# NOC-OI/ship-track-estimators

Hardware: AMD Instinct MI355X
Metric: UKF+URTSS track-steps/sec (dim=4, 500-step tracks) (higher is better)
Workload: dtype f64

## Files before the change

### include/ste.h

```cpp
#ifndef STE_H
#define STE_H

#include <stdint.h>

#ifdef __cplusplus
extern "C" {
#endif

#define STE_VERSION 340

#define STE_OK 0
#define STE_EINVAL (-1)
#define STE_ELAUNCH (-2)
#define STE_ENOGPU (-3)

#define STE_FLAG_SHARED_P0 0x1u
#define STE_FLAG_NO_INITIAL_UPDATE 0x2u
#define STE_FLAG_LANES_1 0x10u
#define STE_FLAG_LANES_4 0x20u
#define STE_FLAG_PACKED_COV 0x40u
#define STE_FLAG_ROBUST 0x4u

#define STE_RTS_WORK_ROWS 30
#define STE_SLICE_ALIGN 64

#define STE_STATUS_NAN 0x1
#define STE_STATUS_CLAMPED 0x2
#define STE_STATUS_NOCONV 0x4
#define STE_STATUS_ROBUST_CAP 0x8
#define STE_STATUS_HOST_INDEX 0x10
#define STE_STATUS_BAD_INDEX 0x20

typedef struct ste_ukf_batch_f64 {
    int32_t B;
    int32_t Nmax;
    int32_t Tmax;
    int32_t n;
    uint32_t flags;
    int32_t tuning;
#define STE_TUNING_EIG_GAINS 0x100
#define STE_TUNING_TWO_KERNEL_SMOOTHER 0x200
#define STE_TUNING_ONE_KERNEL_SMOOTHER 0x400
#define STE_TUNING_LANE_RECURRENCE 0x800

    double fan_scale;
    double w0;
    double wi;

    const double* H;
    const double* Q;
    const double* R;

    const int32_t* nsteps;
    const double* x0;
    const double* P0;

    const double* dt;
    const double* sog_rate;
    const double* cog_rate;
    const double* sog_rate_rts;
    const double* cog_rate_rts;
    const int32_t* upd_idx;
    const double* z;

    const double* noise_pred;
    const double* noise_upd;
    const double* noise_rts;

    double* fwd_mean;
    double* fwd_cov;
    double* sm_mean;
    double* sm_cov;
    int32_t* status;

    double* rts_work;

    double chi_alpha;
    int32_t robust_max_iter;
    int32_t reserved2;

    int64_t track_stride;

    double* sm_pos;

    int32_t step_begin;
    int32_t step_end;
} ste_ukf_batch_f64;

int ste_version(void);

const char* ste_last_error(void);

int ste_device_count(void);

int ste_ukf_forward_f64(const ste_ukf_batch_f64* b, void* stream);

// ... 180 lines not shown
```

### ship-track-estimators_amd/csrc/ste_kernels.hip

```cpp
#include <hip/hip_runtime.h>

#include <algorithm>
#include <cstddef>
#include <cstdint>
#include <cstdio>
#include <cstring>
#include <type_traits>
#include <vector>

#include "../../include/ste.h"
#include "ste_err.h"
#include "ste_ukf.h"
#include "ste_quad.h"

namespace ste {

__shared__ int g_sched_word[2];
__device__ __forceinline__ int sched_k0() { return *(volatile int*)&g_sched_word[0]; }

template <bool kWarm>
__device__ __forceinline__ int sigma_fan(const double (&x)[4], const double (&P)[4][4], double scale,
                                         double (&sig)[9][4], EigBasis& basis);

__device__ __forceinline__ int sigma_fan(const double (&x)[4], const double (&P)[4][4], double scale,
// ... 910 lines not shown
            double Pb[4][4], D[4][4], Pbi[4][4], K[4][4];
            weighted_outer<true>(dk, dk, p.m.w0, p.m.wi, Pb);
            STE_UNROLL
            for (int r = 0; r < 4; ++r) {
                STE_UNROLL
                for (int c = 0; c < 4; ++c) Pb[r][c] += track_Q(r, c);
            }
            weighted_outer<false>(sig0, db, p.m.w0, p.m.wi, D);
            st |= sym_pinv4<true>(Pb, Pbi, pb_basis);
            pb_basis.valid = true;
            mm(D, Pbi, K);
            double y[4];
            STE_UNROLL
            for (int c = 0; c < 4; ++c) y[c] = xs[c] - xb[c];
            y[3] = wrap180(y[3]);
            STE_UNROLL
            for (int r = 0; r < 4; ++r) {
                double acc = xk[r];
                STE_UNROLL
                for (int c = 0; c < 4; ++c) acc = fma(K[r][c], y[c], acc);
                xs[r] = acc;
            }
            xs[3] = floored_mod(xs[3], 360.0);
            double dP[4][4], KdP[4][4], U[4][4];
            STE_UNROLL
            for (int r = 0; r < 4; ++r) {
                STE_UNROLL
                for (int c = 0; c < 4; ++c) dP[r][c] = Ps[r][c] - Pb[r][c];
            }
            mm(K, dP, KdP);
            mmt_sym(KdP, K, U);
            STE_UNROLL
            for (int r = 0; r < 4; ++r) {
                STE_UNROLL
                for (int c = 0; c < 4; ++c) Ps[r][c] = Pk[r][c] + U[r][c];
            }
            store_vec(p.sm_mean, (size_t)k, B, t, xs);
            store_cov_m(p.sm_cov, packed, (size_t)k, B, t, Ps);
            store_pos(p, (size_t)k, B, t, xs);
        }
    }
    if (!all_finite(xs, Ps)) st |= STE_STATUS_NAN;
    if (st) atomicOr(&p.status[t], st);
}

__device__ __forceinline__ bool work_row_full(const KParams& p, int k, int ui, bool always_full) {
    return always_full || (ui >= 0 && ui < p.Tmax) || (k == 0 && !(p.flags & STE_FLAG_NO_INITIAL_UPDATE));
}

struct RecurRow {
    double D2[8], xk[4], Pk[10];
    double shift[2];
};
template <bool kShift>
__device__ __forceinline__ void load_recur_row(const KParams& p, size_t k, size_t B, size_t t, bool d_rows23, RecurRow& g) {
    g.shift[0] = g.shift[1] = 0.0;
    if (kShift) {
        const double dt = p.dt[k * B + t];
        if (p.sog_rate_rts) g.shift[0] = (p.sog_rate_rts[k * B + t] - p.sog_rate[k * B + t]) * dt;
        if (p.cog_rate_rts) g.shift[1] = (p.cog_rate_rts[k * B + t] - p.cog_rate[k * B + t]) * dt;
    }
    const double* w = p.rts_work + (k * kWorkElems) * B + t;
    STE_UNROLL
    for (int e = 0; e < 4; ++e) g.D2[e] = w[(kWorkD + e) * B];
    if (d_rows23) {
        STE_UNROLL
        for (int e = 4; e < 8; ++e) g.D2[e] = w[(kWorkD + e) * B];
    }
    load_vec(p.fwd_mean, k, B, t, g.xk);
    load_cov_p(p.fwd_cov, (p.flags & STE_FLAG_PACKED_COV) != 0, k, B, t, g.Pk);
}

template <bool kShift, bool kTrackNoise = false>
__device__ __forceinline__ int smoother_step_gain(const KParams& p, int k, size_t B, size_t t, const RecurRow& cur,
                                                  const double (&xn)[4], const double (&Pn)[10], bool full, bool always_full,
                                                  bool all_eig, double kappa, double first_bad, double (&xb)[4],
                                                  double (&Pb)[10], double (&K)[4][4], const double* q4 = nullptr) {
    STE_UNROLL
    for (int c = 0; c < 4; ++c) xb[c] = xn[c];
    if (kShift) {
        xb[2] += cur.shift[0];
        xb[3] += cur.shift[1];
    }
    {
        double bv[4];
        STE_UNROLL
        for (int c = 0; c < 4; ++c) bv[c] = xb[c] - cur.xk[c];
        STE_UNROLL
        for (int r = 0; r < 4; ++r) {
            STE_UNROLL
            for (int c = r; c < 4; ++c) Pb[tix(r, c)] = fma(bv[r], bv[c], Pn[tix(r, c)]);
        }
    }
    if (full) {
        const double* w = p.rts_work + ((size_t)k * kWorkElems) * B + t;
        STE_UNROLL
        for (int c = 0; c < 4; ++c) xb[c] = w[(kWorkXb + c) * B];
        STE_UNROLL
        for (int e = 0; e < 10; ++e) Pb[e] = w[(kWorkPb + e) * B];
        if (kShift) {
            double bv[4];
            STE_UNROLL
            for (int c = 0; c < 4; ++c) bv[c] = xb[c] - cur.xk[c];
            if (p.noise_rts) {
                STE_UNROLL
                for (int c = 0; c < 4; ++c) bv[c] -= p.noise_rts[((size_t)k * 4 + c) * B + t];
            }
            const double s2 = cur.shift[0], s3 = cur.shift[1];
            Pb[tix(0, 2)] = fma(bv[0], s2, Pb[tix(0, 2)]);
            Pb[tix(1, 2)] = fma(bv[1], s2, Pb[tix(1, 2)]);
            Pb[tix(0, 3)] = fma(bv[0], s3, Pb[tix(0, 3)]);
            Pb[tix(1, 3)] = fma(bv[1], s3, Pb[tix(1, 3)]);
            Pb[tix(2, 2)] = fma(bv[2] + bv[2] + s2, s2, Pb[tix(2, 2)]);
            Pb[tix(3, 3)] = fma(bv[3] + bv[3] + s3, s3, Pb[tix(3, 3)]);
            Pb[tix(2, 3)] = fma(bv[2], s3, fma(s2, bv[3] + s3, Pb[tix(2, 3)]));
            xb[2] += s2;
            xb[3] += s3;
        }
    }
    double D[4][4];
    STE_UNROLL
    for (int r = 0; r < 4; ++r) {
        D[r][0] = cur.D2[r * 2 + 0];
        D[r][1] = cur.D2[r * 2 + 1];
        D[r][2] = kappa * cur.Pk[tix(r, 2)];
        D[r][3] = kappa * cur.Pk[tix(r, 3)];
    }
    if (!always_full) {
        double bv[4];
        STE_UNROLL
        for (int c = 0; c < 4; ++c) bv[c] = xb[c] - cur.xk[c];
        STE_UNROLL
        for (int r = 2; r < 4; ++r) {
            STE_UNROLL
            for (int c = 0; c < 2; ++c) {
                const double pm = full ? fma(-bv[c], bv[r], Pb[tix(c, r)]) : Pn[tix(c, r)];
                if constexpr (kTrackNoise)
                    D[r][c] = pm - q4[c * 2 + (r - 2)];
                else
                    D[r][c] = pm - p.m.Q[c * 4 + r];
            }
        }
    }
    if (__builtin_expect(__any((double)k >= first_bad), 0)) {
        if ((double)k >= first_bad) {
            const double* w = p.rts_work + ((size_t)k * kWorkElems) * B + t;
            STE_UNROLL
            for (int r = 0; r < 4; ++r) {
                D[r][2] = w[(kWorkD23 + r * 2 + 0) * B];
                D[r][3] = w[(kWorkD23 + r * 2 + 1) * B];
            }
        }
    }
    return smoother_gain(Pb, D, all_eig, K);

}

__device__ __forceinline__ void track_q4(const KParams& p, const NoiseParams& nz, size_t B, size_t t, double (&q4)[4]) {
    STE_UNROLL
    for (int c = 0; c < 2; ++c) {
        STE_UNROLL
        for (int r = 2; r < 4; ++r) q4[c * 2 + (r - 2)] = nz.Q ? nz.Q[(size_t)tix(c, r) * B + t] : p.m.Q[c * 4 + r];
    }
}

template <bool kShift, bool kTrackNoise = false>
__device__ __forceinline__ void smooth_tile_l1(const KParams& p, const size_t t, const NoiseParams* nz = nullptr) {
    const size_t B = (size_t)p.ld;
    if (t >= (size_t)p.B) return;
    double q4[4] = {0.0, 0.0, 0.0, 0.0};
    if constexpr (kTrackNoise) track_q4(p, *nz, B, t, q4);
    const int ns = p.nsteps ? p.nsteps[t] : p.Nmax;
    const bool always_full = p.noise_pred || p.noise_upd || p.noise_rts;
    const bool all_eig = (p.tuning & STE_TUNING_EIG_GAINS) != 0;
    const double kappa = (p.m.wi + p.m.wi) * p.m.fan_scale;
    const double first_bad = p.first_bad[t];
    const int last_row = p.Nmax > 0 ? p.Nmax - 1 : 0;
    auto clampk = [&](int k) -> int { return min(max(k, 0), last_row); };

    double xs[4], Ps[10], xn[4], Pn[10];
    const bool packed = (p.flags & STE_FLAG_PACKED_COV) != 0;
    load_vec(p.fwd_mean, (size_t)ns, B, t, xs);
    load_cov_p(p.fwd_cov, packed, (size_t)ns, B, t, Ps);
    store_vec(p.sm_mean, (size_t)ns, B, t, xs);
    store_cov_p(p.sm_cov, packed, (size_t)ns, B, t, Ps);
    store_pos(p, (size_t)ns, B, t, xs);
    STE_UNROLL
    for (int c = 0; c < 4; ++c) xn[c] = xs[c];
    STE_UNROLL
    for (int e = 0; e < 10; ++e) Pn[e] = Ps[e];

    RecurRow nxt;
    int ui_n = -1;
    if (ns > 0) {
        load_recur_row<kShift>(p, (size_t)(ns - 1), B, t, always_full, nxt);
        ui_n = p.upd_idx[(size_t)(ns - 1) * B + t];
    }
    int st = 0;
    for (int k = p.Nmax - 1; k >= 0; --k) {
        if (!__any(k < ns)) continue;
        if (k < ns) {
            const RecurRow cur = nxt;
            const bool full = work_row_full(p, k, ui_n, always_full);
            double xb[4], Pb[10], K[4][4];
            st |= smoother_step_gain<kShift, kTrackNoise>(p, k, B, t, cur, xn, Pn, full, always_full, all_eig, kappa, first_bad, xb, Pb, K, q4);
            {
                const int kn = clampk(k - 1);
                load_recur_row<kShift>(p, (size_t)kn, B, t, always_full, nxt);
                ui_n = p.upd_idx[(size_t)kn * B + t];
            }
            double y[4];
            STE_UNROLL
            for (int c = 0; c < 4; ++c) y[c] = xs[c] - xb[c];
            y[3] = wrap180(y[3]);
            STE_UNROLL
            for (int r = 0; r < 4; ++r) {
                double acc = cur.xk[r];
                STE_UNROLL
                for (int c = 0; c < 4; ++c) acc = fma(K[r][c], y[c], acc);
                xs[r] = acc;
            }
            xs[3] = floored_mod(xs[3], 360.0);
            double dP[10];
            STE_UNROLL
            for (int e = 0; e < 10; ++e) dP[e] = Ps[e] - Pb[e];
            double KdP[4][4];
            STE_UNROLL
            for (int r = 0; r < 4; ++r) {
                STE_UNROLL
                for (int c = 0; c < 4; ++c) {
                    double acc = K[r][0] * dP[tix(0, c)];
                    STE_UNROLL
                    for (int i = 1; i < 4; ++i) acc = fma(K[r][i], dP[tix(i, c)], acc);
                    KdP[r][c] = acc;
                }
            }
            STE_UNROLL
            for (int r = 0; r < 4; ++r) {
                STE_UNROLL
                for (int c = r; c < 4; ++c) {
                    double acc = KdP[r][0] * K[c][0];
                    STE_UNROLL
                    for (int i = 1; i < 4; ++i) acc = fma(KdP[r][i], K[c][i], acc);
                    Ps[tix(r, c)] = cur.Pk[tix(r, c)] + acc;
                }
            }
            store_vec(p.sm_mean, (size_t)k, B, t, xs);
            store_cov_p(p.sm_cov, packed, (size_t)k, B, t, Ps);
            store_pos(p, (size_t)k, B, t, xs);
            STE_UNROLL
            for (int c = 0; c < 4; ++c) xn[c] = cur.xk[c];
            STE_UNROLL
            for (int e = 0; e < 10; ++e) Pn[e] = cur.Pk[e];
        }
    }
    double chk = 0.0;
    STE_UNROLL
    for (int c = 0; c < 4; ++c) chk += xs[c] * 0.0;
    STE_UNROLL
    for (int e = 0; e < 10; ++e) chk += Ps[e] * 0.0;
    if (!(chk == 0.0)) st |= STE_STATUS_NAN;
    if (st) atomicOr(&p.status[t], st);
}

template <bool kShift>
__global__ __launch_bounds__(64) void urtss_recur_l1(const KParams p) {
    smooth_tile_l1<kShift>(p, (size_t)blockIdx.x * 64 + threadIdx.x);
}
template <bool kShift>
__global__ __launch_bounds__(64) void urtss_recur_tn(const KParams p, const NoiseParams nz) {
    smooth_tile_l1<kShift, true>(p, (size_t)blockIdx.x * 64 + threadIdx.x, &nz);
}

struct SmoothItem {
    int kp;
    int tile;
    int prog;
    int need;
};
struct SmoothSchedParams {
    const KParams* kps;
    const SmoothItem* items;
    const int* progress;
    int* error;
    unsigned long long timeout_ticks;
};
template <bool kShift>
__global__ __launch_bounds__(64) void urtss_recur_sched(const SmoothSchedParams sp) {
    typedef const KParams __attribute__((address_space(4))) ConstKParams;
    const SmoothItem* ip = sp.items + blockIdx.x;
    const int kp = __builtin_amdgcn_readfirstlane(ip->kp), tile = __builtin_amdgcn_readfirstlane(ip->tile);
    const int prog = __builtin_amdgcn_readfirstlane(ip->prog), need = __builtin_amdgcn_readfirstlane(ip->need);
    if (__hip_atomic_load(sp.error, __ATOMIC_RELAXED, __HIP_MEMORY_SCOPE_AGENT) != 0 ||
        !sched_wait(sp.progress + prog, need, sp.timeout_ticks)) {
        if (threadIdx.x == 0) __hip_atomic_store(sp.error, 2, __ATOMIC_RELAXED, __HIP_MEMORY_SCOPE_AGENT);
        return;
    }
    const KParams& p = *(const KParams*)(ConstKParams*)(uintptr_t)(sp.kps + kp);
    smooth_tile_l1<kShift>(p, (size_t)tile * 64 + threadIdx.x);
}



constexpr int kLeanK01 = kWorkD, kLeanK23 = kWorkD23;

template <bool kShift, bool kTrackNoise>
__global__ __launch_bounds__(64) void urtss_gains_all(const KParams p, const NoiseParams nz) {
    const size_t B = (size_t)p.ld;
    const size_t g = (size_t)blockIdx.x * 64 + threadIdx.x;
    if (g >= (size_t)p.B * (size_t)p.Nmax) return;
    const size_t t = g % (size_t)p.B;
    const int k = (int)(g / (size_t)p.B);
    const int ns = p.nsteps ? p.nsteps[t] : p.Nmax;
    if (k >= ns) return;
    const double fb_raw = p.first_bad[t];
    if (fb_raw < 0.0) return;
    const bool always_full = p.noise_pred || p.noise_upd || p.noise_rts;
    const bool all_eig = (p.tuning & STE_TUNING_EIG_GAINS) != 0;
    const double kappa = (p.m.wi + p.m.wi) * p.m.fan_scale;
    const bool packed = (p.flags & STE_FLAG_PACKED_COV) != 0;
    RecurRow cur;
    load_recur_row<kShift>(p, (size_t)k, B, t, always_full, cur);
    double xn[4], Pn[10];
    load_vec(p.fwd_mean, (size_t)k + 1, B, t, xn);
    load_cov_p(p.fwd_cov, packed, (size_t)k + 1, B, t, Pn);
    const bool full = work_row_full(p, k, p.upd_idx[(size_t)k * B + t], always_full);
    double xb[4], Pb[10], K[4][4], q4[4] = {0.0, 0.0, 0.0, 0.0};
    if constexpr (kTrackNoise) track_q4(p, nz, B, t, q4);
    const int st = smoother_step_gain<kShift, kTrackNoise>(p, k, B, t, cur, xn, Pn, full, always_full, all_eig, kappa, fb_raw, xb, Pb, K, q4);
    double* w = p.rts_work + ((size_t)k * kWorkElems) * B + t;
    STE_UNROLL
    for (int r = 0; r < 4; ++r) {
        w[(kLeanK01 + 2 * r + 0) * B] = K[r][0];
        w[(kLeanK01 + 2 * r + 1) * B] = K[r][1];
        w[(kLeanK23 + 2 * r + 0) * B] = K[r][2];
        w[(kLeanK23 + 2 * r + 1) * B] = K[r][3];
    }
    STE_UNROLL
    for (int c = 0; c < 4; ++c) w[(kWorkXb + c) * B] = xb[c];
    STE_UNROLL
    for (int e = 0; e < 10; ++e) w[(kWorkPb + e) * B] = Pb[e];
    if (st) atomicOr(&p.status[t], st);
}

struct LeanRow {
    double K[4][4], xb[4], Pb[10], xk[4], Pk[10];
};
__device__ __forceinline__ void load_lean_row(const KParams& p, size_t k, size_t B, size_t t, bool packed, LeanRow& g) {
    const double* w = p.rts_work + (k * kWorkElems) * B + t;
    STE_UNROLL
    for (int r = 0; r < 4; ++r) {
        g.K[r][0] = w[(kLeanK01 + 2 * r + 0) * B];
// ... 671 lines not shown
        if (kp->noise_rts) kp->noise_rts += r0 * 4 * ld;
        kp->fwd_mean += r0 * 4 * ld;
        kp->fwd_cov += r0 * (packed ? 10 : 16) * ld;
        if (kp->rts_work) kp->rts_work += r0 * STE_RTS_WORK_ROWS * ld;
    }
    return STE_OK;
}

template <class F>
auto with_bool(bool v, F&& f) {
    return v ? f(std::true_type{}) : f(std::false_type{});
}

template <class F>
auto with_forward_variant(const ste::KParams& kp, F&& f) {
    return with_bool(kp.rts_work != nullptr, [&](auto gains) {
        if (kp.fast_upd && kp.m.robust_iters > 0) return f(gains, std::true_type{}, std::true_type{});
        if (kp.fast_upd) return f(gains, std::true_type{}, std::false_type{});
        return f(gains, std::false_type{}, std::false_type{});
    });
}
int forward_variant(const ste::KParams& kp) {
    return with_forward_variant(kp, [](auto gains, auto fast, auto robust) { return gains() | fast() << 1 | robust() << 2; });
}

int launch_forward(const char* fn, const ste::KParams& kp, const ste::LikParams* lp, const ste::NoiseParams* np, hipStream_t s) {
    if (ste::choose_lanes(kp.B, kp.flags) == 4)
        return ste::launch_forward_q4(kp, s);
    const bool hist = kp.fwd_mean != nullptr;
    if (!hist && kp.rts_work) return fail(STE_EINVAL, "%s: rts_work needs the histories", fn);
    const dim3 grid((unsigned)((kp.B + 63) / 64)), block(64);
    const ste::LikParams l0 = lp ? *lp : ste::LikParams{nullptr, nullptr, nullptr, nullptr};
    with_forward_variant(kp, [&](auto gains, auto fast, auto robust) {
        constexpr bool kG = decltype(gains)::value, kF = decltype(fast)::value, kR = decltype(robust)::value;
        auto launch = [&](auto lik) {
            constexpr int kLik = decltype(lik)::value;
            if (np)
                hipLaunchKernelGGL((ste::ukf_forward_tn<kG, kF, kR, kLik>), grid, block, 0, s, kp, l0, *np);
            else if constexpr (kLik != ste::kLikOff)
                hipLaunchKernelGGL((ste::ukf_forward_lik<kG, kF, kR, kLik>), grid, block, 0, s, kp, l0);
            else
                hipLaunchKernelGGL((ste::ukf_forward_l1<kG, kF, kR>), grid, block, 0, s, kp);
        };
        if (!lp)
            launch(std::integral_constant<int, ste::kLikOff>{});
        else if (hist)
            launch(std::integral_constant<int, ste::kLikHist>{});
        else if constexpr (!kG)
            launch(std::integral_constant<int, ste::kLikOnly>{});
    });
    return check_hip(hipGetLastError(), np ? "ukf_forward_tn launch" : lp ? "ukf_forward_lik launch" : "ukf_forward launch");
}

constexpr int kLeanSmootherMaxTracks = 4096;
bool lean_smoother(const ste::KParams& kp) {
    return kp.rts_work && kp.Nmax > 0 && ((kp.tuning & STE_TUNING_TWO_KERNEL_SMOOTHER) || (!(kp.tuning & STE_TUNING_ONE_KERNEL_SMOOTHER) && kp.B <= kLeanSmootherMaxTracks));
}

int launch_backward(const ste::KParams& kp, const ste::NoiseParams* np, hipStream_t s) {
    const dim3 grid((unsigned)((kp.B + 63) / 64)), block(64);
    const bool shift = kp.sog_rate_rts || kp.cog_rate_rts, tn = np && np->Q;
    const ste::NoiseParams nz = tn ? *np : ste::NoiseParams{nullptr, nullptr};
    auto with_shift_tn = [&](auto&& f) { with_bool(shift, [&](auto sh) { with_bool(tn, [&](auto t) { f(sh, t); }); }); };
    if (lean_smoother(kp)) {
        const dim3 ggrid((unsigned)(((size_t)kp.B * (size_t)kp.Nmax + 63) / 64));
        with_shift_tn([&](auto sh, auto t) {
            hipLaunchKernelGGL((ste::urtss_gains_all<decltype(sh)::value, decltype(t)::value>), ggrid, block, 0, s, kp, nz);
        });
        int rc = check_hip(hipGetLastError(), "urtss_gains_all launch");
        if (rc) return rc;
        if (kp.tuning & STE_TUNING_LANE_RECURRENCE)
            hipLaunchKernelGGL(ste::urtss_recur_lean, grid, block, 0, s, kp);
        else
            hipLaunchKernelGGL(ste::urtss_recur_lean_q4, dim3((unsigned)((kp.B + 15) / 16)), block, 0, s, kp);
        return check_hip(hipGetLastError(), "urtss_recur_lean launch");
    }
    if (kp.rts_work) {
        with_shift_tn([&](auto sh, auto t) {
            if constexpr (decltype(t)::value)
                hipLaunchKernelGGL(ste::urtss_recur_tn<decltype(sh)::value>, grid, block, 0, s, kp, nz);
            else
                hipLaunchKernelGGL(ste::urtss_recur_l1<decltype(sh)::value>, grid, block, 0, s, kp);
        });
        return check_hip(hipGetLastError(), "urtss_recur launch");
    }
    with_bool(tn, [&](auto t) { hipLaunchKernelGGL(ste::urtss_backward_l1<decltype(t)::value>, grid, block, 0, s, kp, nz); });
    return check_hip(hipGetLastError(), "urtss_backward launch");
}

int noise_params(const char* fn, const ste_ukf_batch_f64* b, const ste_ukf_noise_f64* nz, ste::NoiseParams* np) {
    if (!b) return fail(STE_EINVAL, "batch pointer is NULL");
    if (!nz) return fail(STE_EINVAL, "%s: the per-track noise (nz) is NULL", fn);
    if (!nz->Q && !nz->R)
        return fail(STE_EINVAL, "%s: nz->Q and nz->R are both NULL: that is the plain call (without the _noise suffix)", fn);
    if (nz->flags & ~(uint32_t)STE_NOISE_R_BLOCK2) return fail(STE_EINVAL, "%s: unknown bits in nz->flags", fn);
    if (b->flags & STE_FLAG_LANES_4)
        return fail(STE_EINVAL, "%s: the quad forward kernel has no per-track noise: STE_FLAG_LANES_4 is refused", fn);
    np->Q = nz->Q;
    np->R = nz->R;
    return STE_OK;
}
void noise_route(const ste_ukf_batch_f64* b, const ste_ukf_noise_f64* nz, ste::KParams* kp) {
    kp->flags |= STE_FLAG_LANES_1;
    if (!nz->R) return;
    bool sel = true;
    for (int r = 0; r < 4; ++r)
        for (int c = 0; c < 4; ++c) sel = sel && b->H[r * 4 + c] == ((r == c && r < 2) ? 1.0 : 0.0);
    kp->fast_upd = sel && (nz->flags & STE_NOISE_R_BLOCK2) != 0;
}

int whole_passes(const char* fn, const ste_ukf_batch_f64* b, const char* why) {
    if (b->step_begin == 0 && (b->step_end == 0 || b->step_end == b->Nmax)) return STE_OK;
    snprintf(g_err, sizeof(g_err), "%s runs whole passes: %s", fn, why);
    return STE_EINVAL;
}

int lik_params(const char* fn, const ste_ukf_batch_f64* b, const ste_ukf_loglik_f64* l, ste::LikParams* lp, bool* hist) {
    if (!l) return fail(STE_EINVAL, "%s: the likelihood outputs (l) are NULL", fn);
    if (!l->loglik) return fail(STE_EINVAL, "%s: l->loglik is required", fn);
    *hist = b->fwd_mean != nullptr;
    if (*hist != (b->fwd_cov != nullptr))
        return fail(STE_EINVAL, "%s: fwd_mean and fwd_cov go together: both (histories) or neither (the likelihood alone)", fn);
    if (!*hist && b->rts_work)
        return fail(STE_EINVAL, "%s: rts_work needs the histories (the smoother reads both); pass fwd_mean and fwd_cov, or no "
                                "rts_work", fn);
    if (b->flags & STE_FLAG_LANES_4)
        return fail(STE_EINVAL, "%s runs the lane-per-track mapping only: STE_FLAG_LANES_4 is refused", fn);
    *lp = {l->loglik, l->dof, l->nupd, l->nis};
    return whole_passes(fn, b, "the likelihood sums over every update, so time slices (step_begin / step_end) are refused");
}

size_t align16(size_t v) { return (v + 15) & ~(size_t)15; }

struct SchedLayout {
    size_t kps, items, progress, total;
// ... 231 lines not shown
    sp.kps = (const ste::KParams*)(dw + lay.kps);
    sp.items = (const ste::SchedItem*)(dw + lay.items);
    sp.nrounds = sc->nrounds;
    sp.nwaves = sc->nwaves;
    sp.progress = (int*)(dw + lay.progress);
    sp.window_done = sc->window_done;
    sp.error = sc->error;
    sp.timeout_ticks = (unsigned long long)((sc->timeout_s > 0 ? sc->timeout_s : 2.0) * 1e8);
    sp.started = sc->started;
    const dim3 grid((unsigned)sc->nwaves), block(64);
    if (!first) return fail(STE_EINVAL, "scheduled forward pass: no kernel variant");
    with_forward_variant(*first, [&](auto gains, auto fast, auto robust) {
        hipLaunchKernelGGL((ste::ukf_forward_sched<decltype(gains)::value, decltype(fast)::value, decltype(robust)::value>), grid, block,
                           0, s, sp);
    });
    return check_hip(hipGetLastError(), "ukf_forward_sched launch");
}

int ste_stream_wait_counter(const int32_t* counter, int32_t need, int32_t* error, double timeout_s, void* stream) {
    if (!counter) return fail(STE_EINVAL, "counter is NULL");
    hipLaunchKernelGGL(ste::sched_gate, dim3(1), dim3(64), 0, (hipStream_t)stream, (const int*)counter, (int)need, (int*)error,
                       (unsigned long long)((timeout_s > 0 ? timeout_s : 2.0) * 1e8));
    return check_hip(hipGetLastError(), "sched_gate launch");
}

size_t ste_ukf_forward_sched_progress_offset(int32_t nwindows, int32_t max_slices, int64_t ntiles_total, int32_t nrounds,
                                             int32_t nwaves) {
    if (nwindows < 0 || max_slices < 0 || ntiles_total < 0 || nrounds < 0 || nwaves < 0) return 0;
    return sched_layout((size_t)nwindows * ((size_t)max_slices * ((size_t)max_slices + 1) / 2), (size_t)nrounds * (size_t)nwaves,
                        (size_t)ntiles_total).progress;
}

size_t ste_urtss_backward_sched_workspace(int32_t nwindows, int64_t ntiles_total) {
    if (nwindows < 0 || ntiles_total < 0) return 0;
    return align16((size_t)nwindows * sizeof(ste::KParams)) + align16((size_t)ntiles_total * sizeof(ste::SmoothItem));
}

int ste_urtss_backward_sched_f64(const ste_bwd_sched_f64* sc, void* stream) {
    if (!sc) return fail(STE_EINVAL, "schedule pointer is NULL");
    if (sc->nwindows < 1 || !sc->windows) return fail(STE_EINVAL, "scheduled smoother: nwindows >= 1 and windows are required");
    if (sc->nitems < 1 || !sc->items) return fail(STE_EINVAL, "scheduled smoother: nitems >= 1 and items are required");
    if (!sc->host_ws || !sc->dev_ws || !sc->progress || !sc->error)
        return fail(STE_EINVAL, "scheduled smoother: host_ws, dev_ws, progress and error are required");
    const int step = sc->slice_steps ? sc->slice_steps : STE_SLICE_ALIGN;
    if (step < STE_SLICE_ALIGN || step % STE_SLICE_ALIGN != 0)
        return fail(STE_EINVAL, "scheduled smoother: slice_steps must be a positive multiple of STE_SLICE_ALIGN (64)");
    const size_t kp_bytes = align16((size_t)sc->nwindows * sizeof(ste::KParams));
    const size_t total = kp_bytes + align16((size_t)sc->nitems * sizeof(ste::SmoothItem));
    if (sc->ws_bytes < total) return fail(STE_EINVAL, "scheduled smoother: workspace too small (ste_urtss_backward_sched_workspace)");
    char* hw = (char*)sc->host_ws;
    ste::KParams* kps = (ste::KParams*)hw;
    std::vector<int> nslices((size_t)sc->nwindows), tile0((size_t)sc->nwindows + 1);
    size_t ntiles = 0;
    int shift = -1;
    for (int w = 0; w < sc->nwindows; ++w) {
        const ste_ukf_batch_f64& b = sc->windows[w];
        if (b.B <= 0 || b.Nmax <= 0) return fail(STE_EINVAL, "scheduled smoother: a window has B <= 0 or Nmax <= 0");
        if (b.step_begin != 0 || b.step_end != 0) return fail(STE_EINVAL, "scheduled smoother: windows must not carry a step range of their own");
        int rc = make_params(&b, true, kps + w);
        if (rc) return rc;
        const ste::KParams& kp = kps[w];
        if (!kp.rts_work || lean_smoother(kp))
            return fail(STE_EINVAL, "scheduled smoother: every window must take the one-kernel smoother (rts_work, more than 4096 tracks or tuning bit 10)");
        const int sh = (kp.sog_rate_rts || kp.cog_rate_rts) ? 1 : 0;
        if (shift >= 0 && sh != shift) return fail(STE_EINVAL, "scheduled smoother: the windows must agree on smoother rates (one kernel runs them all)");
        shift = sh;
        nslices[w] = std::max(1, (b.Nmax + step - 1) / step);
        tile0[w] = (int)ntiles;
        ntiles += ((size_t)b.B + 63) / 64;
        if (ntiles > 0x7fffffff) return fail(STE_EINVAL, "scheduled smoother: too many tiles");
    }
    tile0[sc->nwindows] = (int)ntiles;
    if ((size_t)sc->nitems != ntiles) return fail(STE_EINVAL, "scheduled smoother: items must name every tile of every window once");
    ste::SmoothItem* items = (ste::SmoothItem*)(hw + kp_bytes);
    std::vector<char> seen(ntiles, 0);
    for (int i = 0; i < sc->nitems; ++i) {
        const int w = sc->items[2 * i], t = sc->items[2 * i + 1];
        if (w < 0 || w >= sc->nwindows || t < 0 || t >= tile0[w + 1] - tile0[w])
            return fail(STE_EINVAL, "scheduled smoother: an item names a window or tile that does not exist");
        if (seen[(size_t)(tile0[w] + t)]) return fail(STE_EINVAL, "scheduled smoother: a tile appears twice");
        seen[(size_t)(tile0[w] + t)] = 1;
        items[i].kp = w;
        items[i].tile = t;
        items[i].prog = tile0[w] + t;
        items[i].need = nslices[w];
    }
    hipStream_t s = (hipStream_t)stream;
    char* dw = (char*)sc->dev_ws;
    int rc = upload_table(dw, hw, total, 0, s, "scheduled smoother: table upload");
    if (rc) return rc;
    ste::SmoothSchedParams sp;
    sp.kps = (const ste::KParams*)dw;
    sp.items = (const ste::SmoothItem*)(dw + kp_bytes);
    sp.progress = sc->progress;
    sp.error = sc->error;
    sp.timeout_ticks = (unsigned long long)((sc->timeout_s > 0 ? sc->timeout_s : 2.0) * 1e8);
    if (shift)
        hipLaunchKernelGGL(ste::urtss_recur_sched<true>, dim3((unsigned)sc->nitems), dim3(64), 0, s, sp);
    else
        hipLaunchKernelGGL(ste::urtss_recur_sched<false>, dim3((unsigned)sc->nitems), dim3(64), 0, s, sp);
    return check_hip(hipGetLastError(), "urtss_recur_sched launch");
}

int ste_urtss_backward_f64(const ste_ukf_batch_f64* b, void* stream) {
    ste::KParams kp;
    int rc = make_params(b, true, &kp);
    if (rc) return rc;
    return launch_backward(kp, nullptr, (hipStream_t)stream);
}

int ste_ukf_urtss_f64(const ste_ukf_batch_f64* b, void* stream) {
    const char* fn = "ste_ukf_urtss_f64";
    ste::KParams kp;
    int rc = make_params(b, true, &kp);
    if (rc) return rc;
    rc = whole_passes(fn, b, "time slices go through ste_ukf_forward_f64");
    if (rc) return rc;
    rc = launch_forward(fn, kp, nullptr, nullptr, (hipStream_t)stream);
    if (rc) return rc;
    return launch_backward(kp, nullptr, (hipStream_t)stream);
}

int ste_ukf_forward_noise_f64(const ste_ukf_batch_f64* b, const ste_ukf_noise_f64* nz, const ste_ukf_loglik_f64* l, void* stream) {
    const char* fn = "ste_ukf_forward_noise_f64";
    ste::NoiseParams np;
    int rc = noise_params(fn, b, nz, &np);
    if (rc) return rc;
    ste::LikParams lp;
    bool hist = true;
    if (l) {
        rc = lik_params(fn, b, l, &lp, &hist);
        if (rc) return rc;
    }
    ste::KParams kp;
    rc = make_params(b, false, &kp, hist);
    if (rc) return rc;
    noise_route(b, nz, &kp);
    if (!l) {
        rc = slice_params(b, &kp);
        if (rc) return rc;
    }
    return launch_forward(fn, kp, l ? &lp : nullptr, &np, (hipStream_t)stream);
}

int ste_urtss_backward_noise_f64(const ste_ukf_batch_f64* b, const ste_ukf_noise_f64* nz, void* stream) {
    ste::NoiseParams np;
    int rc = noise_params("ste_urtss_backward_noise_f64", b, nz, &np);
    if (rc) return rc;
    ste::KParams kp;
    rc = make_params(b, true, &kp);
    if (rc) return rc;
    return launch_backward(kp, &np, (hipStream_t)stream);
}
// ... 192 lines not shown
```

### ship-track-estimators_amd/csrc/ste_ukf.h

```cpp
#pragma once
#include <hip/hip_runtime.h>

#include <cstddef>
#include <cstdint>

#include "../../include/ste.h"
#include "ste_math.h"
#include "ste_lane.h"

namespace ste {

struct KParams {
    int B, Nmax, Tmax;
    unsigned flags;
    int tuning;
    int fast_upd;
    Mats m;
    const int32_t* nsteps;
    const double* x0;
    const double* P0;
    const double* dt;
    const double* sog_rate;
    const double* cog_rate;
    const double* sog_rate_rts;
    const double* cog_rate_rts;
    const int32_t* upd_idx;
    const double* z;
    const double* noise_pred;
    const double* noise_upd;
    const double* noise_rts;
    double* fwd_mean;
    double* fwd_cov;
    double* sm_mean;
    double* sm_cov;
    int32_t* status;
    double* rts_work;
    int ld;
    int k0;
    int qpw;
    double* first_bad;
    double* sm_pos;
};

constexpr unsigned kFlagContinue = 0x10000u;

__device__ __forceinline__ int late_k0() {
    typedef const char __attribute__((address_space(4))) * kptr;
    kptr ka = (kptr)__builtin_amdgcn_kernarg_segment_ptr();
    return *(const volatile int __attribute__((address_space(4)))*)(ka + offsetof(KParams, k0));
}

constexpr int kColdEvery = 64;

constexpr int kWorkD = 0, kWorkXb = 8, kWorkPb = 12, kWorkD23 = 22, kWorkElems = STE_RTS_WORK_ROWS;
static_assert(kWorkElems == 30, "include/ste.h: STE_RTS_WORK_ROWS");
constexpr double kNeverBad = 1e300;

__device__ __forceinline__ void load_mat(const double* base, size_t row, size_t B, size_t t, double (&M)[4][4]) {
    STE_UNROLL
    for (int r = 0; r < 4; ++r) {
        STE_UNROLL
        for (int c = 0; c < 4; ++c) M[r][c] = base[(row * 16 + r * 4 + c) * B + t];
    }
}
__device__ __forceinline__ void st_stream(double* p, double v) { __builtin_nontemporal_store(v, p); }
__device__ __forceinline__ void store_mat(double* base, size_t row, size_t B, size_t t, const double (&M)[4][4]) {
    STE_UNROLL
    for (int r = 0; r < 4; ++r) {
        STE_UNROLL
        for (int c = 0; c < 4; ++c) st_stream(&base[(row * 16 + r * 4 + c) * B + t], M[r][c]);
    }
}
__device__ __forceinline__ void load_vec(const double* base, size_t row, size_t B, size_t t, double (&v)[4]) {
    STE_UNROLL
    for (int c = 0; c < 4; ++c) v[c] = base[(row * 4 + c) * B + t];
}
__device__ __forceinline__ void store_vec(double* base, size_t row, size_t B, size_t t, const double (&v)[4]) {
    STE_UNROLL
    for (int c = 0; c < 4; ++c) st_stream(&base[(row * 4 + c) * B + t], v[c]);
}

__device__ __forceinline__ size_t cov_at(bool packed, size_t row, int r, int c) {
    return packed ? row * 10 + (size_t)(r * 4 - (r * (r - 1)) / 2 + (c - r)) : row * 16 + (size_t)(r * 4 + c);
}
__device__ __forceinline__ void store_cov_p(double* base, bool packed, size_t row, size_t B, size_t t, const double (&P)[10]) {
    STE_UNROLL
    for (int r = 0; r < 4; ++r) {
        STE_UNROLL
        for (int c = r; c < 4; ++c) st_stream(&base[cov_at(packed, row, r, c) * B + t], P[tix(r, c)]);
    }
    if (!packed) {
        STE_UNROLL
        for (int r = 1; r < 4; ++r) {
            STE_UNROLL
            for (int c = 0; c < r; ++c) st_stream(&base[(row * 16 + r * 4 + c) * B + t], P[tix(r, c)]);
        }
    }
}
__device__ __forceinline__ void load_cov_p(const double* base, bool packed, size_t row, size_t B, size_t t, double (&P)[10]) {
    STE_UNROLL
    for (int r = 0; r < 4; ++r) {
        STE_UNROLL
        for (int c = r; c < 4; ++c) P[tix(r, c)] = base[cov_at(packed, row, r, c) * B + t];
    }
}
__device__ __forceinline__ void store_cov_m(double* base, bool packed, size_t row, size_t B, size_t t, const double (&M)[4][4]) {
    STE_UNROLL
    for (int r = 0; r < 4; ++r) {
        STE_UNROLL
        for (int c = 0; c < 4; ++c) {
            if (c >= r)
                st_stream(&base[cov_at(packed, row, r, c) * B + t], M[r][c]);
            else if (!packed)
                st_stream(&base[(row * 16 + r * 4 + c) * B + t], M[r][c]);
        }
    }
}
__device__ __forceinline__ void load_cov_m(const double* base, bool packed, size_t row, size_t B, size_t t, double (&M)[4][4]) {
    STE_UNROLL
    for (int r = 0; r < 4; ++r) {
        STE_UNROLL
        for (int c = 0; c < 4; ++c) {
            if (packed)
                M[r][c] = base[cov_at(true, row, r < c ? r : c, r < c ? c : r) * B + t];
            else
                M[r][c] = base[(row * 16 + r * 4 + c) * B + t];
        }
    }
}

__device__ __forceinline__ bool all_finite(const double (&x)[4], const double (&P)[4][4]) {
    double acc = 0.0;
    STE_UNROLL
    for (int r = 0; r < 4; ++r) {
        acc += x[r] * 0.0;
        STE_UNROLL
        for (int c = 0; c < 4; ++c) acc += P[r][c] * 0.0;
    }
    return acc == 0.0;
}

}
```

### ship-track-estimators_amd/track_estimators/_hip/binding.py

```python
from __future__ import annotations

import ctypes as C
import os

_HERE = os.path.dirname(os.path.abspath(__file__))
PKG_ROOT = os.path.dirname(os.path.dirname(_HERE))
LIB_PATH = os.environ.get("STE_LIB_PATH") or os.path.join(PKG_ROOT, "lib", "libste_hip.so")

STE_FLAG_SHARED_P0 = 0x1
STE_FLAG_NO_INITIAL_UPDATE = 0x2
STE_FLAG_ROBUST = 0x4
STE_FLAG_LANES_1 = 0x10
STE_FLAG_LANES_4 = 0x20
STE_FLAG_PACKED_COV = 0x40

STE_TUNING_EIG_GAINS = 0x100
STE_TUNING_TWO_KERNEL_SMOOTHER = 0x200
STE_TUNING_ONE_KERNEL_SMOOTHER = 0x400
STE_TUNING_LANE_RECURRENCE = 0x800

STE_NOISE_R_BLOCK2 = 0x1

STE_RTS_WORK_ROWS = 30
STE_SLICE_ALIGN = 64

STE_STATUS_NAN = 0x1
STE_STATUS_CLAMPED = 0x2
STE_STATUS_NOCONV = 0x4
STE_STATUS_ROBUST_CAP = 0x8
STE_STATUS_HOST_INDEX = 0x10
STE_STATUS_BAD_INDEX = 0x20

_dp = C.c_void_p


class SteUkfBatchF64(C.Structure):

    _fields_ = [
        ("B", C.c_int32),
        ("Nmax", C.c_int32),
        ("Tmax", C.c_int32),
        ("n", C.c_int32),
        ("flags", C.c_uint32),
        ("tuning", C.c_int32),
        ("fan_scale", C.c_double),
        ("w0", C.c_double),
        ("wi", C.c_double),
        ("H", _dp),
        ("Q", _dp),
        ("R", _dp),
        ("nsteps", _dp),
        ("x0", _dp),
        ("P0", _dp),
        ("dt", _dp),
        ("sog_rate", _dp),
        ("cog_rate", _dp),
        ("sog_rate_rts", _dp),
        ("cog_rate_rts", _dp),
        ("upd_idx", _dp),
        ("z", _dp),
        ("noise_pred", _dp),
        ("noise_upd", _dp),
        ("noise_rts", _dp),
        ("fwd_mean", _dp),
        ("fwd_cov", _dp),
        ("sm_mean", _dp),
        ("sm_cov", _dp),
        ("status", _dp),
        ("rts_work", _dp),
        ("chi_alpha", C.c_double),
        ("robust_max_iter", C.c_int32),
        ("reserved2", C.c_int32),
# ... 214 lines not shown
```

Measured before the change: 7.907 billion.

## Address smoother rows through AMD buffer resources with scalar row pointers

```diff
diff --git a/include/ste.h b/include/ste.h
--- a/include/ste.h
+++ b/include/ste.h
@@ -42,6 +42,7 @@
 #define STE_TUNING_TWO_KERNEL_SMOOTHER 0x200
 #define STE_TUNING_ONE_KERNEL_SMOOTHER 0x400
 #define STE_TUNING_LANE_RECURRENCE 0x800
+#define STE_TUNING_FLAT_ADDRESSING 0x1000
 
     double fan_scale;
     double w0;
diff --git a/ship-track-estimators_amd/csrc/ste_kernels.hip b/ship-track-estimators_amd/csrc/ste_kernels.hip
--- a/ship-track-estimators_amd/csrc/ste_kernels.hip
+++ b/ship-track-estimators_amd/csrc/ste_kernels.hip
@@ -986,14 +986,56 @@
     double D2[8], xk[4], Pk[10];
     double shift[2];
 };
-template <bool kShift>
-__device__ __forceinline__ void load_recur_row(const KParams& p, size_t k, size_t B, size_t t, bool d_rows23, RecurRow& g) {
+struct SmoothRows {
+    RowBuf xbpb, sm_mean, sm_cov, sm_pos;
+    RowBuf work_a, mean_a, cov_a, upd_a;
+    RowOffs o;
+    __device__ __forceinline__ void init(const KParams& p, size_t t) {
+        const unsigned ld = (unsigned)p.ld, n = (unsigned)p.Nmax;
+        const unsigned ce = (p.flags & STE_FLAG_PACKED_COV) ? 10u : 16u;
+        o.init(t, ld);
+        xbpb.init(p.rts_work + (size_t)kWorkXb * ld, n, kWorkElems, ld, 8);
+        sm_mean.init(p.sm_mean, n, 4, ld, 8);
+        sm_cov.init(p.sm_cov, n, ce, ld, 8);
+        sm_pos.init(p.sm_pos, n, 2, ld, 8);
+        work_a.init(p.rts_work, n - 1, kWorkElems, ld, 8);
+        mean_a.init(p.fwd_mean, n - 1, 4, ld, 8);
+        cov_a.init(p.fwd_cov, n - 1, ce, ld, 8);
+        upd_a.init(p.upd_idx, n - 1, 1, ld, 4);
+    }
+    __device__ __forceinline__ void step(int k) {
+        xbpb.prev(xbpb.pitch);
+        sm_mean.prev(sm_mean.pitch);
+        sm_cov.prev(sm_cov.pitch);
+        sm_pos.prev(sm_pos.pitch);
+        const bool mv = k > 0;
+        work_a.prev(mv ? work_a.pitch : 0u);
+        mean_a.prev(mv ? mean_a.pitch : 0u);
+        cov_a.prev(mv ? cov_a.pitch : 0u);
+        upd_a.prev(mv ? upd_a.pitch : 0u);
+    }
+};
+
+template <bool kShift, bool kBuf = false>
+__device__ __forceinline__ void load_recur_row(const KParams& p, size_t k, size_t B, size_t t, bool d_rows23, RecurRow& g,
+                                               const SmoothRows* rw = nullptr) {
     g.shift[0] = g.shift[1] = 0.0;
     if (kShift) {
         const double dt = p.dt[k * B + t];
         if (p.sog_rate_rts) g.shift[0] = (p.sog_rate_rts[k * B + t] - p.sog_rate[k * B + t]) * dt;
         if (p.cog_rate_rts) g.shift[1] = (p.cog_rate_rts[k * B + t] - p.cog_rate[k * B + t]) * dt;
     }
+    if constexpr (kBuf) {
+        STE_UNROLL
+        for (int e = 0; e < 4; ++e) g.D2[e] = rw->work_a.load(rw->o, (unsigned)(kWorkD + e));
+        if (d_rows23) {
+            STE_UNROLL
+            for (int e = 4; e < 8; ++e) g.D2[e] = rw->work_a.load(rw->o, (unsigned)(kWorkD + e));
+        }
+        load_vec(rw->mean_a, rw->o, g.xk);
+        load_cov_p(rw->cov_a, (p.flags & STE_FLAG_PACKED_COV) != 0, rw->o, g.Pk);
+        return;
+    }
     const double* w = p.rts_work + (k * kWorkElems) * B + t;
     STE_UNROLL
     for (int e = 0; e < 4; ++e) g.D2[e] = w[(kWorkD + e) * B];
@@ -1005,11 +1047,12 @@
     load_cov_p(p.fwd_cov, (p.flags & STE_FLAG_PACKED_COV) != 0, k, B, t, g.Pk);
 }
 
-template <bool kShift, bool kTrackNoise = false>
+template <bool kShift, bool kTrackNoise = false, bool kBuf = false>
 __device__ __forceinline__ int smoother_step_gain(const KParams& p, int k, size_t B, size_t t, const RecurRow& cur,
                                                   const double (&xn)[4], const double (&Pn)[10], bool full, bool always_full,
                                                   bool all_eig, double kappa, double first_bad, double (&xb)[4],
-                                                  double (&Pb)[10], double (&K)[4][4], const double* q4 = nullptr) {
+                                                  double (&Pb)[10], double (&K)[4][4], const double* q4 = nullptr,
+                                                  const SmoothRows* rw = nullptr) {
     STE_UNROLL
     for (int c = 0; c < 4; ++c) xb[c] = xn[c];
     if (kShift) {
@@ -1027,11 +1070,18 @@
         }
     }
     if (full) {
-        const double* w = p.rts_work + ((size_t)k * kWorkElems) * B + t;
-        STE_UNROLL
-        for (int c = 0; c < 4; ++c) xb[c] = w[(kWorkXb + c) * B];
-        STE_UNROLL
-        for (int e = 0; e < 10; ++e) Pb[e] = w[(kWorkPb + e) * B];
+        if constexpr (kBuf) {
+            STE_UNROLL
+            for (int c = 0; c < 4; ++c) xb[c] = rw->xbpb.load(rw->o, (unsigned)(kWorkXb - kWorkXb + c));
+            STE_UNROLL
+            for (int e = 0; e < 10; ++e) Pb[e] = rw->xbpb.load(rw->o, (unsigned)(kWorkPb - kWorkXb + e));
+        } else {
+            const double* w = p.rts_work + ((size_t)k * kWorkElems) * B + t;
+            STE_UNROLL
+            for (int c = 0; c < 4; ++c) xb[c] = w[(kWorkXb + c) * B];
+            STE_UNROLL
+            for (int e = 0; e < 10; ++e) Pb[e] = w[(kWorkPb + e) * B];
+        }
         if (kShift) {
             double bv[4];
             STE_UNROLL
@@ -1098,7 +1148,7 @@
     }
 }
 
-template <bool kShift, bool kTrackNoise = false>
+template <bool kShift, bool kTrackNoise = false, bool kBuf = false>
 __device__ __forceinline__ void smooth_tile_l1(const KParams& p, const size_t t, const NoiseParams* nz = nullptr) {
     const size_t B = (size_t)p.ld;
     if (t >= (size_t)p.B) return;
@@ -1131,14 +1181,20 @@
         ui_n = p.upd_idx[(size_t)(ns - 1) * B + t];
     }
     int st = 0;
+    SmoothRows rw;
+    if constexpr (kBuf) rw.init(p, t);
     for (int k = p.Nmax - 1; k >= 0; --k) {
+        if constexpr (kBuf) rw.step(k);
         if (!__any(k < ns)) continue;
         if (k < ns) {
             const RecurRow cur = nxt;
             const bool full = work_row_full(p, k, ui_n, always_full);
             double xb[4], Pb[10], K[4][4];
-            st |= smoother_step_gain<kShift, kTrackNoise>(p, k, B, t, cur, xn, Pn, full, always_full, all_eig, kappa, first_bad, xb, Pb, K, q4);
-            {
+            st |= smoother_step_gain<kShift, kTrackNoise, kBuf>(p, k, B, t, cur, xn, Pn, full, always_full, all_eig, kappa, first_bad, xb, Pb, K, q4, &rw);
+            if constexpr (kBuf) {
+                load_recur_row<kShift, true>(p, (size_t)clampk(k - 1), B, t, always_full, nxt, &rw);
+                ui_n = rw.upd_a.load_i32(rw.o);
+            } else {
                 const int kn = clampk(k - 1);
                 load_recur_row<kShift>(p, (size_t)kn, B, t, always_full, nxt);
                 ui_n = p.upd_idx[(size_t)kn * B + t];
@@ -1179,9 +1235,18 @@
                     Ps[tix(r, c)] = cur.Pk[tix(r, c)] + acc;
                 }
             }
-            store_vec(p.sm_mean, (size_t)k, B, t, xs);
-            store_cov_p(p.sm_cov, packed, (size_t)k, B, t, Ps);
-            store_pos(p, (size_t)k, B, t, xs);
+            if constexpr (kBuf) {
+                store_vec(rw.sm_mean, rw.o, xs);
+                store_cov_p(rw.sm_cov, packed, rw.o, Ps);
+                if (p.sm_pos) {
+                    rw.sm_pos.store_nt(rw.o, 0, xs[0]);
+                    rw.sm_pos.store_nt(rw.o, 1, xs[1]);
+                }
+            } else {
+                store_vec(p.sm_mean, (size_t)k, B, t, xs);
+                store_cov_p(p.sm_cov, packed, (size_t)k, B, t, Ps);
+                store_pos(p, (size_t)k, B, t, xs);
+            }
             STE_UNROLL
             for (int c = 0; c < 4; ++c) xn[c] = cur.xk[c];
             STE_UNROLL
@@ -1197,13 +1262,13 @@
     if (st) atomicOr(&p.status[t], st);
 }
 
-template <bool kShift>
+template <bool kShift, bool kBuf>
 __global__ __launch_bounds__(64) void urtss_recur_l1(const KParams p) {
-    smooth_tile_l1<kShift>(p, (size_t)blockIdx.x * 64 + threadIdx.x);
-}
-template <bool kShift>
+    smooth_tile_l1<kShift, false, kBuf>(p, (size_t)blockIdx.x * 64 + threadIdx.x);
+}
+template <bool kShift, bool kBuf>
 __global__ __launch_bounds__(64) void urtss_recur_tn(const KParams p, const NoiseParams nz) {
-    smooth_tile_l1<kShift, true>(p, (size_t)blockIdx.x * 64 + threadIdx.x, &nz);
+    smooth_tile_l1<kShift, true, kBuf>(p, (size_t)blockIdx.x * 64 + threadIdx.x, &nz);
 }
 
 struct SmoothItem {
@@ -1219,7 +1284,7 @@
     int* error;
     unsigned long long timeout_ticks;
 };
-template <bool kShift>
+template <bool kShift, bool kBuf>
 __global__ __launch_bounds__(64) void urtss_recur_sched(const SmoothSchedParams sp) {
     typedef const KParams __attribute__((address_space(4))) ConstKParams;
     const SmoothItem* ip = sp.items + blockIdx.x;
@@ -1231,7 +1296,7 @@
         return;
     }
     const KParams& p = *(const KParams*)(ConstKParams*)(uintptr_t)(sp.kps + kp);
-    smooth_tile_l1<kShift>(p, (size_t)tile * 64 + threadIdx.x);
+    smooth_tile_l1<kShift, false, kBuf>(p, (size_t)tile * 64 + threadIdx.x);
 }
 
 
@@ -2009,6 +2074,10 @@
     return check_hip(hipGetLastError(), np ? "ukf_forward_tn launch" : lp ? "ukf_forward_lik launch" : "ukf_forward launch");
 }
 
+bool buffer_rows(const ste::KParams& kp) {
+    return !(kp.tuning & STE_TUNING_FLAT_ADDRESSING) && kp.ld <= ste::kBufMaxLd && !(kp.sog_rate_rts || kp.cog_rate_rts);
+}
+
 constexpr int kLeanSmootherMaxTracks = 4096;
 bool lean_smoother(const ste::KParams& kp) {
     return kp.rts_work && kp.Nmax > 0 && ((kp.tuning & STE_TUNING_TWO_KERNEL_SMOOTHER) || (!(kp.tuning & STE_TUNING_ONE_KERNEL_SMOOTHER) && kp.B <= kLeanSmootherMaxTracks));
@@ -2034,10 +2103,13 @@
     }
     if (kp.rts_work) {
         with_shift_tn([&](auto sh, auto t) {
-            if constexpr (decltype(t)::value)
-                hipLaunchKernelGGL(ste::urtss_recur_tn<decltype(sh)::value>, grid, block, 0, s, kp, nz);
-            else
-                hipLaunchKernelGGL(ste::urtss_recur_l1<decltype(sh)::value>, grid, block, 0, s, kp);
+            with_bool(buffer_rows(kp), [&](auto buf) {
+                constexpr bool kSh = decltype(sh)::value, kBuf = decltype(buf)::value && !kSh;
+                if constexpr (decltype(t)::value)
+                    hipLaunchKernelGGL((ste::urtss_recur_tn<kSh, kBuf>), grid, block, 0, s, kp, nz);
+                else
+                    hipLaunchKernelGGL((ste::urtss_recur_l1<kSh, kBuf>), grid, block, 0, s, kp);
+            });
         });
         return check_hip(hipGetLastError(), "urtss_recur launch");
     }
@@ -2375,7 +2447,7 @@
     ste::KParams* kps = (ste::KParams*)hw;
     std::vector<int> nslices((size_t)sc->nwindows), tile0((size_t)sc->nwindows + 1);
     size_t ntiles = 0;
-    int shift = -1;
+    int shift = -1, buf = -1;
     for (int w = 0; w < sc->nwindows; ++w) {
         const ste_ukf_batch_f64& b = sc->windows[w];
         if (b.B <= 0 || b.Nmax <= 0) return fail(STE_EINVAL, "scheduled smoother: a window has B <= 0 or Nmax <= 0");
@@ -2388,6 +2460,10 @@
         const int sh = (kp.sog_rate_rts || kp.cog_rate_rts) ? 1 : 0;
         if (shift >= 0 && sh != shift) return fail(STE_EINVAL, "scheduled smoother: the windows must agree on smoother rates (one kernel runs them all)");
         shift = sh;
+        const int bf = buffer_rows(kp) ? 1 : 0;
+        if (buf >= 0 && bf != buf)
+            return fail(STE_EINVAL, "scheduled smoother: the windows must agree on how rows are addressed (tuning bit 12, or a track_stride above 17 895 697)");
+        buf = bf;
         nslices[w] = std::max(1, (b.Nmax + step - 1) / step);
         tile0[w] = (int)ntiles;
         ntiles += ((size_t)b.B + 63) / 64;
@@ -2418,10 +2494,12 @@
     sp.progress = sc->progress;
     sp.error = sc->error;
     sp.timeout_ticks = (unsigned long long)((sc->timeout_s > 0 ? sc->timeout_s : 2.0) * 1e8);
-    if (shift)
-        hipLaunchKernelGGL(ste::urtss_recur_sched<true>, dim3((unsigned)sc->nitems), dim3(64), 0, s, sp);
-    else
-        hipLaunchKernelGGL(ste::urtss_recur_sched<false>, dim3((unsigned)sc->nitems), dim3(64), 0, s, sp);
+    with_bool(shift != 0, [&](auto sh) {
+        with_bool(buf != 0, [&](auto bf) {
+            constexpr bool kSh = decltype(sh)::value, kBuf = decltype(bf)::value && !kSh;
+            hipLaunchKernelGGL((ste::urtss_recur_sched<kSh, kBuf>), dim3((unsigned)sc->nitems), dim3(64), 0, s, sp);
+        });
+    });
     return check_hip(hipGetLastError(), "urtss_recur_sched launch");
 }
 
diff --git a/ship-track-estimators_amd/csrc/ste_ukf.h b/ship-track-estimators_amd/csrc/ste_ukf.h
--- a/ship-track-estimators_amd/csrc/ste_ukf.h
+++ b/ship-track-estimators_amd/csrc/ste_ukf.h
@@ -56,6 +56,54 @@
 static_assert(kWorkElems == 30, "include/ste.h: STE_RTS_WORK_ROWS");
 constexpr double kNeverBad = 1e300;
 
+typedef unsigned buf_v2u __attribute__((ext_vector_type(2)));
+constexpr int kBufWord3 = 0x00020000;
+constexpr int kBufNt = 2;
+constexpr int kBufMaxLd = (int)(0xffffffffu / (STE_RTS_WORK_ROWS * 8u));
+constexpr int kBufScalarElems = 8, kBufMaxElems = 16;
+struct RowOffs {
+    unsigned vo, ld8;
+    unsigned vhi[kBufMaxElems - kBufScalarElems];
+    __device__ __forceinline__ void init(size_t t, unsigned ld) {
+        vo = (unsigned)t * 8u;
+        ld8 = ld * 8u;
+        STE_UNROLL
+        for (int i = 0; i < kBufMaxElems - kBufScalarElems; ++i) {
+            unsigned v = vo + (unsigned)(kBufScalarElems + i) * ld8;
+            asm volatile("" : "+v"(v));
+            vhi[i] = v;
+        }
+    }
+    __device__ __forceinline__ unsigned v(unsigned e) const { return e < (unsigned)kBufScalarElems ? vo : vhi[e - kBufScalarElems]; }
+    __device__ __forceinline__ unsigned s(unsigned e) const { return e < (unsigned)kBufScalarElems ? e * ld8 : 0u; }
+};
+struct RowBuf {
+    unsigned lo, hi;
+    unsigned pitch;
+    __device__ __forceinline__ void init(const void* a, unsigned row, unsigned elems, unsigned ld, unsigned esize) {
+        pitch = elems * ld * esize;
+        const uintptr_t u = (uintptr_t)a + (size_t)row * pitch;
+        lo = __builtin_amdgcn_readfirstlane((unsigned)u);
+        hi = __builtin_amdgcn_readfirstlane((unsigned)(u >> 32));
+    }
+    __device__ __forceinline__ void prev(unsigned by) { asm("s_sub_u32 %0, %0, %2\n\ts_subb_u32 %1, %1, 0" : "+s"(lo), "+s"(hi) : "s"(by) : "scc"); }
+    __device__ __forceinline__ __amdgpu_buffer_rsrc_t rsrc() const {
+        return __builtin_amdgcn_make_buffer_rsrc((void*)((uintptr_t)lo | ((uintptr_t)hi << 32)), 0, (int)pitch, kBufWord3);
+    }
+    __device__ __forceinline__ double load(const RowOffs& o, unsigned e) const {
+        return __builtin_bit_cast(double, __builtin_amdgcn_raw_buffer_load_b64(rsrc(), (int)o.v(e), (int)o.s(e), 0));
+    }
+    __device__ __forceinline__ void store_nt(const RowOffs& o, unsigned e, double v) const {
+        __builtin_amdgcn_raw_buffer_store_b64(__builtin_bit_cast(buf_v2u, v), rsrc(), (int)o.v(e), (int)o.s(e), kBufNt);
+    }
+    __device__ __forceinline__ int load_i32(const RowOffs& o) const {
+        return (int)__builtin_amdgcn_raw_buffer_load_b32(rsrc(), (int)(o.vo >> 1), 0, 0);
+    }
+};
+__device__ __forceinline__ unsigned cov_elem(bool packed, int r, int c) {
+    return packed ? (unsigned)(r * 4 - (r * (r - 1)) / 2 + (c - r)) : (unsigned)(r * 4 + c);
+}
+
 __device__ __forceinline__ void load_mat(const double* base, size_t row, size_t B, size_t t, double (&M)[4][4]) {
     STE_UNROLL
     for (int r = 0; r < 4; ++r) {
@@ -102,6 +150,35 @@
     for (int r = 0; r < 4; ++r) {
         STE_UNROLL
         for (int c = r; c < 4; ++c) P[tix(r, c)] = base[cov_at(packed, row, r, c) * B + t];
+    }
+}
+__device__ __forceinline__ void load_vec(const RowBuf& b, const RowOffs& o, double (&v)[4]) {
+    STE_UNROLL
+    for (int c = 0; c < 4; ++c) v[c] = b.load(o, (unsigned)c);
+}
+__device__ __forceinline__ void store_vec(const RowBuf& b, const RowOffs& o, const double (&v)[4]) {
+    STE_UNROLL
+    for (int c = 0; c < 4; ++c) b.store_nt(o, (unsigned)c, v[c]);
+}
+__device__ __forceinline__ void store_cov_p(const RowBuf& b, bool packed, const RowOffs& o, const double (&P)[10]) {
+    STE_UNROLL
+    for (int r = 0; r < 4; ++r) {
+        STE_UNROLL
+        for (int c = r; c < 4; ++c) b.store_nt(o, cov_elem(packed, r, c), P[tix(r, c)]);
+    }
+    if (!packed) {
+        STE_UNROLL
+        for (int r = 1; r < 4; ++r) {
+            STE_UNROLL
+            for (int c = 0; c < r; ++c) b.store_nt(o, (unsigned)(r * 4 + c), P[tix(r, c)]);
+        }
+    }
+}
+__device__ __forceinline__ void load_cov_p(const RowBuf& b, bool packed, const RowOffs& o, double (&P)[10]) {
+    STE_UNROLL
+    for (int r = 0; r < 4; ++r) {
+        STE_UNROLL
+        for (int c = r; c < 4; ++c) P[tix(r, c)] = b.load(o, cov_elem(packed, r, c));
     }
 }
 __device__ __forceinline__ void store_cov_m(double* base, bool packed, size_t row, size_t B, size_t t, const double (&M)[4][4]) {
diff --git a/ship-track-estimators_amd/track_estimators/_hip/binding.py b/ship-track-estimators_amd/track_estimators/_hip/binding.py
--- a/ship-track-estimators_amd/track_estimators/_hip/binding.py
+++ b/ship-track-estimators_amd/track_estimators/_hip/binding.py
@@ -18,6 +18,7 @@
 STE_TUNING_TWO_KERNEL_SMOOTHER = 0x200
 STE_TUNING_ONE_KERNEL_SMOOTHER = 0x400
 STE_TUNING_LANE_RECURRENCE = 0x800
+STE_TUNING_FLAT_ADDRESSING = 0x1000
 
 STE_NOISE_R_BLOCK2 = 0x1
 
```

Result: no change. 7.935 billion, median of 6 (+0.3%).
